# Emilianogith/MPC-for-dynamic-locomotion-in-the-MIT-cheetah-3

Measured on AMD Instinct MI355X. Metric: QP solves/sec (horizon=10, 4-contact Lite3) at batch=4096, higher is better.
Workload: dtype f32 tiles + f64 residuals

## Files before the change

mpc-for-dynamic-locomotion-in-the-mit-cheetah-3_amd/csrc/mpcqp_common.h:

```cpp
#pragma once
#include "mpcqp_device.h"

namespace {

typedef float f2 __attribute__((ext_vector_type(2)));
__device__ __forceinline__ f2 mk2(float a, float b) { f2 t = {a, b}; return t; }
__device__ __forceinline__ f2 splat2(float v) { return mk2(v, v); }

template <typename TIO>
struct FastIn {
  const TIO* x0; const TIO* r; const uint8_t* contact; const TIO* xdes; const TIO* mu;
  const TIO* ref; const TIO* feet0; const TIO* footholds; const int32_t* gait; const uint8_t* feet_id;
  const TIO* u_init;
  float* y_state;
  int shift;
};

template <typename TIO>
__device__ __forceinline__ double xdes_elem(const TIO* rf, const TIO g, const int k, const int c, const double d, const double gate) {
  if (c < 2) return (double)rf[c];
  if (c == 2) return (double)rf[2] + (double)k * d * gate * (double)rf[9];
  if (c < 6) return (double)rf[c] + (double)k * d * gate * (double)rf[6 + (c - 3)];
  if (c < 8) return 0.0;
  if (c == 8) return gate * (double)rf[9];
  if (c < 12) return gate * (double)rf[6 + (c - 9)];
  return (double)g;
}

template <typename TF, typename TIO>
__device__ __forceinline__ double lever_elem(const TF foot, const TIO* rf, const TIO* x, const int k, const int a, const double d,
                                             const double gate) {
  const double com = k == 0 ? (double)x[3 + a] : (double)rf[3 + a] + (double)k * d * gate * (double)rf[6 + a];
  return (double)foot - com;
}

constexpr int MODEL_ROW = 6;


#ifndef MPCQP_HARD_ITER_FACTOR
#define MPCQP_HARD_ITER_FACTOR 2
#endif
constexpr int ADAPT_AT = 25;
constexpr float ADAPT_RHO_MAX = 30.f;
constexpr double ALPHA_EASY = 1e-2;
constexpr int HARD_ITER_FACTOR = MPCQP_HARD_ITER_FACTOR;
constexpr int HARD_POLISH_FACTOR = 2;
#ifndef MPCQP_WARM_POLISH
#define MPCQP_WARM_POLISH 2
#endif
constexpr int WARM_POLISH = MPCQP_WARM_POLISH;
#ifndef MPCQP_WARM_K
#define MPCQP_WARM_K 60
#endif
constexpr int WARM_K = MPCQP_WARM_K;
#ifndef MPCQP_WARM_FRAC10
#define MPCQP_WARM_FRAC10 4
#endif
constexpr int WARM_FRAC10 = MPCQP_WARM_FRAC10;
constexpr float WARM_KKT_TOL = 1e-3f;

constexpr int ORDER_BUCKETS = 16;
struct OrderBuf { int* cnt; int* list; int cap; int* head; int* zero; };

__device__ __forceinline__ float support_demand(int nst, const float (&fx)[4], const float (&fy)[4], const float (&fz)[4],
                                                const bool (&st)[4]) {
  if (nst == 2) {
    int a = -1, bidx = -1;
#pragma unroll
    for (int l = 0; l < 4; ++l) { if (st[l]) { if (a < 0) a = l; else bidx = l; } }
    const float dx = fx[a] - fx[bidx], dy = fy[a] - fy[bidx];
    const float d = fabsf(fx[a] * fy[bidx] - fy[a] * fx[bidx]) / fmaxf(sqrtf(dx * dx + dy * dy), 1e-6f);
    const float h = fmaxf(-0.5f * (fz[a] + fz[bidx]), 1e-3f);
    return d / h;
  }
  if (nst == 1) {
#pragma unroll
    for (int l = 0; l < 4; ++l) if (st[l]) return sqrtf(fx[l] * fx[l] + fy[l] * fy[l]) / fmaxf(-fz[l], 1e-3f);
  }
  return 0.f;
}

__device__ __forceinline__ int cost_class(float nst, float demand_over_mu) {
  const float us = 2.2f * nst + 34.f * fminf(demand_over_mu, 2.f);
  return isfinite(us) ? (int)fminf(us * 0.1f, (float)(ORDER_BUCKETS - 1)) : 0;
}

template <typename TIO, int N>
__global__ void __launch_bounds__(1024)
mpcqp_order_kernel(const FastIn<TIO> in, const int B, const OrderBuf ob) {
  __shared__ int lcnt[ORDER_BUCKETS], lbase[ORDER_BUCKETS];
  if (threadIdx.x < ORDER_BUCKETS) lcnt[threadIdx.x] = 0;
  if (blockIdx.x == 0 && threadIdx.x < 32 && ob.zero) ob.zero[threadIdx.x] = 0;
  __syncthreads();
  const int b = blockIdx.x * 64 + (threadIdx.x >> 4), k0 = threadIdx.x & 15;
  float score = 0.f, cnt = 0.f;
  for (int k = k0; k < N && b < B; k += 16) {
    float fx[4], fy[4], fz[4]; bool st[4]; int nst = 0;
#pragma unroll
    for (int l = 0; l < 4; ++l) {
      const TIO* rp = in.r + ((size_t)b * N + k) * 12 + 3 * l;
      fx[l] = (float)rp[0]; fy[l] = (float)rp[1]; fz[l] = (float)rp[2];
      st[l] = in.contact[((size_t)b * N + k) * 4 + l] != 0;
      nst += st[l] ? 1 : 0;
    }
    float sc = support_demand(nst, fx, fy, fz, st);
    if (!isfinite(sc)) sc = 0.f;
    score = fmaxf(score, sc);
    cnt += (float)nst;
  }
  score = fmaxf(score, dpp_mov<0xB1>(score));
  score = fmaxf(score, dpp_mov<0x4E>(score));
  score = fmaxf(score, dpp_mov<0x141>(score));
  score = fmaxf(score, dpp_mov<0x140>(score));
  cnt += dpp_mov<0xB1>(cnt);
  cnt += dpp_mov<0x4E>(cnt);
  cnt += dpp_mov<0x141>(cnt);
  cnt += dpp_mov<0x140>(cnt);
  int bucket = 0, pos = 0;
  const bool filer = b < B && k0 == 0;
  if (filer) {
    bucket = cost_class(cnt * (10.f / N), score / fmaxf(fabsf((float)in.mu[b]), 1e-3f));
    pos = atomicAdd(&lcnt[bucket], 1);
  }
  __syncthreads();
  if (threadIdx.x < ORDER_BUCKETS) lbase[threadIdx.x] = lcnt[threadIdx.x] ? atomicAdd(&ob.cnt[threadIdx.x], lcnt[threadIdx.x]) : 0;
  __syncthreads();
  if (filer) ob.list[(size_t)bucket * ob.cap + lbase[bucket] + pos] = b;
}

}
```

Baseline: 12.52 million.

## Replace order-kernel cost heuristic with fitted logistic classifier and ballot-based bucketing

Replaces the cost-class heuristic that sorts batch elements into work buckets. The new score is a fitted linear model over per-stage contact masks, saturation runs, friction demand and horizontal velocity error. The aim is to group problems of similar iteration count so the solver wastes fewer divergent iterations. The shared-memory atomics and two syncthreads for bucket placement are replaced with wave ballots and a single atomic per class. The kernel now also reads xdes and x0, and the fitted coefficients may not carry over to other input distributions.

```diff
diff --git a/mpc-for-dynamic-locomotion-in-the-mit-cheetah-3_amd/csrc/mpcqp_common.h b/mpc-for-dynamic-locomotion-in-the-mit-cheetah-3_amd/csrc/mpcqp_common.h
--- a/mpc-for-dynamic-locomotion-in-the-mit-cheetah-3_amd/csrc/mpcqp_common.h
+++ b/mpc-for-dynamic-locomotion-in-the-mit-cheetah-3_amd/csrc/mpcqp_common.h
@@ -1,5 +1,6 @@
 #pragma once
 #include "mpcqp_device.h"
+#include "mpcqp_order.h"
 
 namespace {
 
@@ -59,73 +60,75 @@
 constexpr int WARM_FRAC10 = MPCQP_WARM_FRAC10;
 constexpr float WARM_KKT_TOL = 1e-3f;
 
-constexpr int ORDER_BUCKETS = 16;
 struct OrderBuf { int* cnt; int* list; int cap; int* head; int* zero; };
-
-__device__ __forceinline__ float support_demand(int nst, const float (&fx)[4], const float (&fy)[4], const float (&fz)[4],
-                                                const bool (&st)[4]) {
-  if (nst == 2) {
-    int a = -1, bidx = -1;
-#pragma unroll
-    for (int l = 0; l < 4; ++l) { if (st[l]) { if (a < 0) a = l; else bidx = l; } }
-    const float dx = fx[a] - fx[bidx], dy = fy[a] - fy[bidx];
-    const float d = fabsf(fx[a] * fy[bidx] - fy[a] * fx[bidx]) / fmaxf(sqrtf(dx * dx + dy * dy), 1e-6f);
-    const float h = fmaxf(-0.5f * (fz[a] + fz[bidx]), 1e-3f);
-    return d / h;
-  }
-  if (nst == 1) {
-#pragma unroll
-    for (int l = 0; l < 4; ++l) if (st[l]) return sqrtf(fx[l] * fx[l] + fy[l] * fy[l]) / fmaxf(-fz[l], 1e-3f);
-  }
-  return 0.f;
-}
-
-__device__ __forceinline__ int cost_class(float nst, float demand_over_mu) {
-  const float us = 2.2f * nst + 34.f * fminf(demand_over_mu, 2.f);
-  return isfinite(us) ? (int)fminf(us * 0.1f, (float)(ORDER_BUCKETS - 1)) : 0;
-}
+static_assert(ORDER_BUCKETS + 1 <= 32, "class counters and the queue head share a header set of 32 ints");
 
 template <typename TIO, int N>
 __global__ void __launch_bounds__(1024)
 mpcqp_order_kernel(const FastIn<TIO> in, const int B, const OrderBuf ob) {
-  __shared__ int lcnt[ORDER_BUCKETS], lbase[ORDER_BUCKETS];
-  if (threadIdx.x < ORDER_BUCKETS) lcnt[threadIdx.x] = 0;
+  static_assert(N <= 32, "one mask bit per stage");
+  __shared__ int lcls[64];
   if (blockIdx.x == 0 && threadIdx.x < 32 && ob.zero) ob.zero[threadIdx.x] = 0;
-  __syncthreads();
-  const int b = blockIdx.x * 64 + (threadIdx.x >> 4), k0 = threadIdx.x & 15;
-  float score = 0.f, cnt = 0.f;
-  for (int k = k0; k < N && b < B; k += 16) {
-    float fx[4], fy[4], fz[4]; bool st[4]; int nst = 0;
+  const int q = threadIdx.x >> 4, b = blockIdx.x * 64 + q, k0 = threadIdx.x & 15, row = 16 * (q & 3);
+  const bool live = b < B;
+  float inv_mu = 0.f, vx = 0.f, vy = 0.f;
+  bool bad = false;
+  if (live) {
+    const float mu = (float)in.mu[b];
+    bad = !isfinite(mu);
+    inv_mu = 1.f / fmaxf(fabsf(mu), 1e-3f);
+    vx = (float)in.x0[(size_t)b * 13 + 9]; vy = (float)in.x0[(size_t)b * 13 + 10];
+  }
+  uint32_t two = 0, sat = 0;
+  float dmax = 0.f, hvmax = 0.f, cnt = 0.f;
 #pragma unroll
-    for (int l = 0; l < 4; ++l) {
-      const TIO* rp = in.r + ((size_t)b * N + k) * 12 + 3 * l;
-      fx[l] = (float)rp[0]; fy[l] = (float)rp[1]; fz[l] = (float)rp[2];
-      st[l] = in.contact[((size_t)b * N + k) * 4 + l] != 0;
-      nst += st[l] ? 1 : 0;
+  for (int p = 0; p < (N + 15) / 16; ++p) {
+    const int k = k0 + 16 * p;
+    OrderStage s = {0.f, 0.f, 0.f, false, false, false};
+    if (live && k < N) {
+      float r[12]; bool ct[4];
+      const TIO* rp = in.r + ((size_t)b * N + k) * 12;
+#pragma unroll
+      for (int i = 0; i < 12; ++i) r[i] = (float)rp[i];
+#pragma unroll
+      for (int l = 0; l < 4; ++l) ct[l] = in.contact[((size_t)b * N + k) * 4 + l] != 0;
+      const TIO* xk = in.xdes + ((size_t)b * (N + 1) + k + 1) * 13;
+      s = order_stage(r, ct, vx - (float)xk[9], vy - (float)xk[10], inv_mu);
     }
-    float sc = support_demand(nst, fx, fy, fz, st);
-    if (!isfinite(sc)) sc = 0.f;
-    score = fmaxf(score, sc);
-    cnt += (float)nst;
+    const unsigned long long m2 = __ballot(s.two), ms = __ballot(s.sat), mb = __ballot(s.bad);
+    two |= (uint32_t)((m2 >> row) & 0xffffu) << (16 * p);
+    sat |= (uint32_t)((ms >> row) & 0xffffu) << (16 * p);
+    bad = bad || ((mb >> row) & 0xffffu) != 0;
+    dmax = fmaxf(dmax, s.demand); hvmax = fmaxf(hvmax, s.hv); cnt += s.nst;
   }
-  score = fmaxf(score, dpp_mov<0xB1>(score));
-  score = fmaxf(score, dpp_mov<0x4E>(score));
-  score = fmaxf(score, dpp_mov<0x141>(score));
-  score = fmaxf(score, dpp_mov<0x140>(score));
+  dmax = fmaxf(dmax, dpp_mov<0xB1>(dmax));
+  dmax = fmaxf(dmax, dpp_mov<0x4E>(dmax));
+  dmax = fmaxf(dmax, dpp_mov<0x141>(dmax));
+  dmax = fmaxf(dmax, dpp_mov<0x140>(dmax));
+  hvmax = fmaxf(hvmax, dpp_mov<0xB1>(hvmax));
+  hvmax = fmaxf(hvmax, dpp_mov<0x4E>(hvmax));
+  hvmax = fmaxf(hvmax, dpp_mov<0x141>(hvmax));
+  hvmax = fmaxf(hvmax, dpp_mov<0x140>(hvmax));
   cnt += dpp_mov<0xB1>(cnt);
   cnt += dpp_mov<0x4E>(cnt);
   cnt += dpp_mov<0x141>(cnt);
   cnt += dpp_mov<0x140>(cnt);
-  int bucket = 0, pos = 0;
-  const bool filer = b < B && k0 == 0;
-  if (filer) {
-    bucket = cost_class(cnt * (10.f / N), score / fmaxf(fabsf((float)in.mu[b]), 1e-3f));
-    pos = atomicAdd(&lcnt[bucket], 1);
+  if (k0 == 0) lcls[q] = live ? cost_class(N, two, sat, cnt, dmax, hvmax, bad) : -1;
+  __syncthreads();
+  if (threadIdx.x < 64) {
+    const int lane = threadIdx.x, cls = lcls[lane];
+    int pos = 0, mine = 0;
+#pragma unroll
+    for (int c = 0; c < ORDER_BUCKETS; ++c) {
+      const unsigned long long m = __ballot(cls == c);
+      if (cls == c) pos = __popcll(m & ((1ull << lane) - 1ull));
+      if (lane == c) mine = __popcll(m);
+    }
+    int base = 0;
+    if (lane < ORDER_BUCKETS && mine) base = atomicAdd(&ob.cnt[lane], mine);
+    base = __shfl(base, cls < 0 ? 0 : cls);
+    if (cls >= 0) ob.list[(size_t)cls * ob.cap + base + pos] = blockIdx.x * 64 + lane;
   }
-  __syncthreads();
-  if (threadIdx.x < ORDER_BUCKETS) lbase[threadIdx.x] = lcnt[threadIdx.x] ? atomicAdd(&ob.cnt[threadIdx.x], lcnt[threadIdx.x]) : 0;
-  __syncthreads();
-  if (filer) ob.list[(size_t)bucket * ob.cap + lbase[bucket] + pos] = b;
 }
 
 }
diff --git a/mpc-for-dynamic-locomotion-in-the-mit-cheetah-3_amd/csrc/mpcqp_order.h b/mpc-for-dynamic-locomotion-in-the-mit-cheetah-3_amd/csrc/mpcqp_order.h
--- /dev/null
+++ b/mpc-for-dynamic-locomotion-in-the-mit-cheetah-3_amd/csrc/mpcqp_order.h
@@ -0,0 +1,89 @@
+#pragma once
+#include <cmath>
+#include <cstdint>
+
+#if defined(__HIPCC__) || defined(__CUDACC__)
+#define ORDER_FN __host__ __device__ __forceinline__
+#else
+#define ORDER_FN inline
+#endif
+
+namespace {
+
+constexpr int ORDER_BUCKETS = 16;
+
+ORDER_FN float support_demand(int nst, const float (&fx)[4], const float (&fy)[4], const float (&fz)[4], const bool (&st)[4]) {
+  if (nst == 2) {
+    int a = -1, bidx = -1;
+    for (int l = 0; l < 4; ++l) { if (st[l]) { if (a < 0) a = l; else bidx = l; } }
+    const float dx = fx[a] - fx[bidx], dy = fy[a] - fy[bidx];
+    const float n2 = dx * dx + dy * dy, cr = fabsf(fx[a] * fy[bidx] - fy[a] * fx[bidx]), hz = -0.5f * (fz[a] + fz[bidx]);
+    if (!std::isfinite(n2 + cr + fabsf(hz))) return NAN;
+    return cr / fmaxf(sqrtf(n2), 1e-6f) / fmaxf(hz, 1e-3f);
+  }
+  if (nst == 1) {
+    for (int l = 0; l < 4; ++l) {
+      if (!st[l]) continue;
+      const float n2 = fx[l] * fx[l] + fy[l] * fy[l];
+      if (!std::isfinite(n2 + fabsf(fz[l]))) return NAN;
+      return sqrtf(n2) / fmaxf(-fz[l], 1e-3f);
+    }
+  }
+  return 0.f;
+}
+
+struct OrderStage {
+  float nst;
+  float demand;
+  float hv;
+  bool two;
+  bool sat;
+  bool bad;
+};
+ORDER_FN OrderStage order_stage(const float (&r)[12], const bool (&ct)[4], float evx, float evy, float inv_mu) {
+  float fx[4], fy[4], fz[4];
+  int nst = 0;
+  for (int l = 0; l < 4; ++l) { fx[l] = r[3 * l]; fy[l] = r[3 * l + 1]; fz[l] = r[3 * l + 2]; nst += ct[l] ? 1 : 0; }
+  OrderStage s;
+  s.nst = (float)nst;
+  s.demand = support_demand(nst, fx, fy, fz, ct) * inv_mu;
+  s.hv = sqrtf(evx * evx + evy * evy) * inv_mu;
+  s.two = nst == 1 || nst == 2;
+  s.bad = !(std::isfinite(s.demand) && std::isfinite(s.hv));
+  s.sat = s.two && s.demand > 1.f;
+  return s;
+}
+
+ORDER_FN int order_ctz(uint32_t v) { return v ? __builtin_ctz(v) : 32; }
+ORDER_FN int order_popc(uint32_t v) { return __builtin_popcount(v); }
+
+ORDER_FN int cost_class(int N, uint32_t two, uint32_t sat, float nst_sum, float dmax, float hvmax, bool bad) {
+#ifdef MPCQP_ORDER_ROUND1
+  const float us = 2.2f * (nst_sum * (10.f / (float)N)) + 34.f * fminf(dmax, 2.f);
+  return (!bad && std::isfinite(us)) ? (int)fminf(us * 0.1f, (float)(ORDER_BUCKETS - 1)) : 0;
+#endif
+  const uint32_t all = N >= 32 ? 0xffffffffu : ((1u << N) - 1u);
+  two &= all; sat &= all;
+  const int lead = order_ctz(~sat);
+  int s = order_ctz(two); if (s > N) s = N;
+  const uint32_t from_s = s < 32 ? (two >> s) : 0u;
+  const int L = order_ctz(~from_s);
+  const uint32_t run = (L >= 32 ? 0xffffffffu : ((1u << L) - 1u)) << (s < 32 ? s : 0);
+  const int nsat = order_popc(sat & run);
+  const float late = s >= 1 ? ldexpf((float)L, 1 - s) : 0.f;
+  const float late_sat = late * (float)nsat / (float)(L > 1 ? L : 1);
+  const float has_late = (s >= 1 && L >= 1) ? 1.f : 0.f;
+  const float swing10 = 40.f - nst_sum * (10.f / (float)N);
+  float z = -9.2251f;
+  z += 1.0399f * (float)(lead < 6 ? lead : 6);
+  z += 1.0684f * fminf(dmax, 2.f);
+  z += 0.14989f * late;
+  z += 0.11830f * late_sat;
+  z += 1.1557f * hvmax;
+  z += 2.2787f * has_late;
+  z += -0.013650f * swing10;
+  if (bad || !std::isfinite(z)) return 0;
+  return (int)fminf(fmaxf((z + 9.5f) * 2.f, 0.f), (float)(ORDER_BUCKETS - 1));
+}
+
+}
```

Measured after the change: 14.91 million, median of 6. 19.1% higher.
